# kyle-wedgwood/ArmadilloCUDALinearInterpolation

Hardware: NVIDIA B200
Metric: interp points/s (2-D bilinear, 4096x4096 f64 grid, 1e8 scattered queries) (higher is better)
Workload: dtype f64

## Files before the change

armadillocudalinearinterpolation_b200/csrc/host_staging.cuh:

```cuda
#pragma once
#include <cstdlib>
#include <cstring>
#include <string>
#include <thread>
#include <vector>
#include "common.cuh"

namespace b200 {

inline bool host_pageable(const void* p) {
  if (!p) return false;
  cudaPointerAttributes a;
  if (cudaPointerGetAttributes(&a, p) != cudaSuccess) { cudaGetLastError(); return true; }
  return a.type == cudaMemoryTypeUnregistered;
}

struct StageArray { const void* in; void* out; size_t elem; };

struct StagePool {
  static constexpr int kSlots = 2;
  struct Worker {
    cudaStream_t st = nullptr;
    cudaEvent_t ev[kSlots] = {nullptr, nullptr};
    std::vector<void*> pin[kSlots], dev[kSlots];
  };
  std::vector<Worker> workers;
  std::vector<size_t> elems;
  size_t chunk = 0;
  int device = -1;

  void release() {
    if (device >= 0) cudaSetDevice(device);
    for (Worker& w : workers) {
      for (int s = 0; s < kSlots; ++s) {
        for (void* p : w.pin[s]) cudaFreeHost(p);
        for (void* p : w.dev[s]) cudaFree(p);
        if (w.ev[s]) cudaEventDestroy(w.ev[s]);
      }
      if (w.st) cudaStreamDestroy(w.st);
    }
    workers.clear(); elems.clear(); chunk = 0;
  }
  ~StagePool() { release(); }

  int ensure(int dev_id, int nworkers, size_t chunk_elems, const std::vector<StageArray>& arrays) {
    bool same = device == dev_id && (int)workers.size() == nworkers && chunk == chunk_elems && elems.size() == arrays.size();
    for (size_t a = 0; same && a < arrays.size(); ++a) same = elems[a] == arrays[a].elem;
    if (same) return B200_OK;
    release();
    const int rc = build(dev_id, nworkers, chunk_elems, arrays);
    if (rc != B200_OK) release();
    return rc;
  }

  int build(int dev_id, int nworkers, size_t chunk_elems, const std::vector<StageArray>& arrays) {
    device = dev_id;
    chunk = chunk_elems;
    for (const StageArray& a : arrays) elems.push_back(a.elem);
    workers.resize(nworkers);
    for (Worker& w : workers) {
      B200_CUDA(cudaStreamCreateWithFlags(&w.st, cudaStreamNonBlocking));
      for (int s = 0; s < kSlots; ++s) {
        B200_CUDA(cudaEventCreateWithFlags(&w.ev[s], cudaEventDisableTiming));
        for (size_t e : elems) {
          void *hp = nullptr, *dp = nullptr;
          B200_CUDA(cudaHostAlloc(&hp, chunk * e, cudaHostAllocDefault));
          w.pin[s].push_back(hp);
          B200_CUDA(cudaMalloc(&dp, chunk * e));
          w.dev[s].push_back(dp);
        }
      }
    }
    return B200_OK;
  }
};

template <class Launch>
int staged_run(StagePool& pool, int device, const std::vector<StageArray>& arrays, size_t n, Launch launch) {
  if (n == 0) return B200_OK;
  constexpr size_t kChunkElems = (size_t)1 << 20;
  unsigned hw = std::thread::hardware_concurrency();
  int nworkers = (int)(hw >= 16 ? 8 : (hw >= 4 ? hw / 2 : 1));
  const size_t nchunks = (n + kChunkElems - 1) / kChunkElems;
  if ((size_t)nworkers > nchunks) nworkers = (int)nchunks;
  B200_TRY(pool.ensure(device, nworkers, kChunkElems, arrays));
  std::vector<int> status(nworkers, B200_OK);
  std::vector<std::string> text(nworkers);
  auto body = [&](int t) {
    auto run = [&]() -> int {
      B200_CUDA(cudaSetDevice(device));
      StagePool::Worker& w = pool.workers[t];
      bool pending[StagePool::kSlots] = {false, false};
      size_t p_off[StagePool::kSlots] = {0, 0}, p_cnt[StagePool::kSlots] = {0, 0};
      auto drain = [&](int s) -> int {
        if (!pending[s]) return B200_OK;
        B200_CUDA(cudaEventSynchronize(w.ev[s]));
        for (size_t a = 0; a < arrays.size(); ++a)
          if (arrays[a].out) memcpy((char*)arrays[a].out + p_off[s] * arrays[a].elem, w.pin[s][a], p_cnt[s] * arrays[a].elem);
        pending[s] = false;
        return B200_OK;
      };
      int slot = 0;
      for (size_t c = (size_t)t; c < nchunks; c += (size_t)nworkers, slot ^= 1) {
        const size_t off = c * kChunkElems, cnt = n - off < kChunkElems ? n - off : kChunkElems;
        B200_TRY(drain(slot));
        NvtxRange nvtx_chunk("staged:chunk memcpy+h2d+kernel+d2h");
        for (size_t a = 0; a < arrays.size(); ++a)
          if (arrays[a].in) {
            memcpy(w.pin[slot][a], (const char*)arrays[a].in + off * arrays[a].elem, cnt * arrays[a].elem);
            B200_CUDA(cudaMemcpyAsync(w.dev[slot][a], w.pin[slot][a], cnt * arrays[a].elem, cudaMemcpyHostToDevice, w.st));
          }
        B200_TRY(launch(w.dev[slot], cnt, w.st));
        for (size_t a = 0; a < arrays.size(); ++a)
          if (arrays[a].out)
            B200_CUDA(cudaMemcpyAsync(w.pin[slot][a], w.dev[slot][a], cnt * arrays[a].elem, cudaMemcpyDeviceToHost, w.st));
        B200_CUDA(cudaEventRecord(w.ev[slot], w.st));
        pending[slot] = true; p_off[slot] = off; p_cnt[slot] = cnt;
      }
      for (int s = 0; s < StagePool::kSlots; ++s) B200_TRY(drain(s));
      return B200_OK;
    };
    status[t] = run();
    if (status[t] != B200_OK) text[t] = b200_last_error();
  };
  std::vector<std::thread> th;
  bool spawn_failed = false;
  try {
    for (int t = 1; t < nworkers; ++t) th.emplace_back(body, t);
  } catch (...) {
    spawn_failed = true;
  }
  body(0);
  for (std::thread& x : th) x.join();
  if (spawn_failed) return fail(B200_ERR_CUDA, "staged copy: could not start the worker threads");
  for (int t = 0; t < nworkers; ++t)
    if (status[t] != B200_OK) return fail(status[t], "%s", text[t].c_str());
  return B200_OK;
}

}
```

Before: 55.91 billion.

## Replace per-call staging threads with persistent piece-scheduled pool and streaming copies

Replaces the per-call spawning of worker threads, each owning two slots, with a persistent thread pool. The pool shares six slots, each with its own stream, and splits chunks into pieces scheduled by a state machine (in, gpu, out), using cudaLaunchHostFunc callbacks to mark GPU completion. Host copies into and out of pinned buffers use AVX2/SSE2 non-temporal stores, and the thread count follows CPU affinity up to 16. This aims to remove thread creation cost and to overlap the host memcpy, the PCIe transfers and the kernels more fully. In exchange it adds mutex and condition-variable contention, a std::function call per launch, and considerable scheduling complexity.

Result: no change. 55.90 billion, median of 6 (-0.0%).

```diff
diff --git a/armadillocudalinearinterpolation_b200/csrc/host_staging.cuh b/armadillocudalinearinterpolation_b200/csrc/host_staging.cuh
--- a/armadillocudalinearinterpolation_b200/csrc/host_staging.cuh
+++ b/armadillocudalinearinterpolation_b200/csrc/host_staging.cuh
@@ -1,9 +1,16 @@
 #pragma once
+#include <sched.h>
+#include <condition_variable>
 #include <cstdlib>
 #include <cstring>
+#include <functional>
+#include <mutex>
 #include <string>
 #include <thread>
 #include <vector>
+#if defined(__x86_64__)
+#include <immintrin.h>
+#endif
 #include "common.cuh"
 
 namespace b200 {
@@ -15,61 +22,311 @@
   return a.type == cudaMemoryTypeUnregistered;
 }
 
+#if defined(__x86_64__)
+__attribute__((target("avx2"))) inline void stream_body_avx2(char* d, const char* s, size_t n) {
+  for (; n; n -= 128, d += 128, s += 128) {
+    const __m256i a = _mm256_loadu_si256((const __m256i*)s), b = _mm256_loadu_si256((const __m256i*)(s + 32)),
+                  c = _mm256_loadu_si256((const __m256i*)(s + 64)), e = _mm256_loadu_si256((const __m256i*)(s + 96));
+    _mm256_stream_si256((__m256i*)d, a);
+    _mm256_stream_si256((__m256i*)(d + 32), b);
+    _mm256_stream_si256((__m256i*)(d + 64), c);
+    _mm256_stream_si256((__m256i*)(d + 96), e);
+  }
+}
+inline void stream_body_sse2(char* d, const char* s, size_t n) {
+  for (; n; n -= 64, d += 64, s += 64) {
+    const __m128i a = _mm_loadu_si128((const __m128i*)s), b = _mm_loadu_si128((const __m128i*)(s + 16)),
+                  c = _mm_loadu_si128((const __m128i*)(s + 32)), e = _mm_loadu_si128((const __m128i*)(s + 48));
+    _mm_stream_si128((__m128i*)d, a);
+    _mm_stream_si128((__m128i*)(d + 16), b);
+    _mm_stream_si128((__m128i*)(d + 32), c);
+    _mm_stream_si128((__m128i*)(d + 48), e);
+  }
+}
+#endif
+
+inline void stream_copy(void* dst, const void* src, size_t n) {
+#if defined(__x86_64__)
+  static const bool avx2 = (__builtin_cpu_init(), __builtin_cpu_supports("avx2"));
+  char* d = (char*)dst;
+  const char* s = (const char*)src;
+  const size_t head = (32 - ((uintptr_t)d & 31)) & 31;
+  if (n < head + 128) { memcpy(d, s, n); return; }
+  memcpy(d, s, head);
+  d += head; s += head; n -= head;
+  const size_t body = n & ~(size_t)127;
+  if (avx2) stream_body_avx2(d, s, body);
+  else stream_body_sse2(d, s, body);
+  memcpy(d + body, s + body, n - body);
+#else
+  memcpy(dst, src, n);
+#endif
+}
+inline void stream_fence() {
+#if defined(__x86_64__)
+  _mm_sfence();
+#endif
+}
+
+inline int affinity_cpus() {
+  cpu_set_t set;
+  if (sched_getaffinity(0, sizeof(set), &set) == 0) return CPU_COUNT(&set);
+  const unsigned hw = std::thread::hardware_concurrency();
+  return hw ? (int)hw : 1;
+}
+
 struct StageArray { const void* in; void* out; size_t elem; };
 
+using StageLaunch = std::function<int(const std::vector<void*>&, size_t, cudaStream_t)>;
+
 struct StagePool {
-  static constexpr int kSlots = 2;
-  struct Worker {
-    cudaStream_t st = nullptr;
-    cudaEvent_t ev[kSlots] = {nullptr, nullptr};
-    std::vector<void*> pin[kSlots], dev[kSlots];
+  int max_threads = 16;
+  int nslots = 6;
+  size_t chunk_elems = (size_t)2 << 20;
+  size_t piece_elems = (size_t)1 << 19;
+
+  struct Slot { cudaStream_t st = nullptr; void* pin = nullptr; void* dev = nullptr; };
+  std::vector<Slot> slots;
+  size_t slot_bytes = 0;
+  int device = -1;
+
+  enum { kFree, kIn, kGpu, kOut };
+  struct Run { size_t chunk = 0, off = 0, cnt = 0; int state = kFree, pieces = 0, in_given = 0, in_done = 0,
+               out_given = 0, out_done = 0; };
+  struct Job;
+  struct Done { StagePool* pool; Job* job; int slot; };
+  struct Job {
+    const std::vector<StageArray>* arrays;
+    size_t n, nchunks;
+    int device;
+    const StageLaunch* launch;
+    std::vector<size_t> offs;
+    std::vector<Run> run;
+    std::vector<Done> done;
+    size_t next_chunk = 0, chunks_done = 0;
+    int status = B200_OK;
+    std::string text;
   };
-  std::vector<Worker> workers;
-  std::vector<size_t> elems;
-  size_t chunk = 0;
-  int device = -1;
-
+  enum { kTaskNone, kTaskIn, kTaskOut };
+  struct Task { int kind = kTaskNone, slot = 0, piece = 0; };
+
+  std::vector<std::thread> threads;
+  std::mutex mu;
+  std::condition_variable cv;
+  Job* job = nullptr;
+  unsigned long long job_id = 0;
+  int busy = 0;
+  bool quit = false;
+
+  StagePool() = default;
+  StagePool(const StagePool&) = delete;
+  StagePool& operator=(const StagePool&) = delete;
+  ~StagePool() { release(); }
+
+  void join_threads() {
+    {
+      std::lock_guard<std::mutex> lk(mu);
+      quit = true;
+    }
+    cv.notify_all();
+    for (std::thread& t : threads) t.join();
+    threads.clear();
+    quit = false;
+  }
+  void free_slots() {
+    if (device >= 0) cudaSetDevice(device);
+    for (Slot& s : slots) {
+      if (s.st) cudaStreamSynchronize(s.st);
+      if (s.pin) cudaFreeHost(s.pin);
+      if (s.dev) cudaFree(s.dev);
+      if (s.st) cudaStreamDestroy(s.st);
+    }
+    slots.clear();
+    slot_bytes = 0;
+  }
   void release() {
-    if (device >= 0) cudaSetDevice(device);
-    for (Worker& w : workers) {
-      for (int s = 0; s < kSlots; ++s) {
-        for (void* p : w.pin[s]) cudaFreeHost(p);
-        for (void* p : w.dev[s]) cudaFree(p);
-        if (w.ev[s]) cudaEventDestroy(w.ev[s]);
-      }
-      if (w.st) cudaStreamDestroy(w.st);
-    }
-    workers.clear(); elems.clear(); chunk = 0;
-  }
-  ~StagePool() { release(); }
-
-  int ensure(int dev_id, int nworkers, size_t chunk_elems, const std::vector<StageArray>& arrays) {
-    bool same = device == dev_id && (int)workers.size() == nworkers && chunk == chunk_elems && elems.size() == arrays.size();
-    for (size_t a = 0; same && a < arrays.size(); ++a) same = elems[a] == arrays[a].elem;
-    if (same) return B200_OK;
-    release();
-    const int rc = build(dev_id, nworkers, chunk_elems, arrays);
-    if (rc != B200_OK) release();
+    join_threads();
+    free_slots();
+  }
+
+  int ensure_slots(int dev_id, size_t bytes) {
+    if (device == dev_id && (int)slots.size() == nslots && slot_bytes >= bytes) return B200_OK;
+    free_slots();
+    device = dev_id;
+    const int rc = build_slots(bytes);
+    if (rc != B200_OK) free_slots();
     return rc;
   }
-
-  int build(int dev_id, int nworkers, size_t chunk_elems, const std::vector<StageArray>& arrays) {
-    device = dev_id;
-    chunk = chunk_elems;
-    for (const StageArray& a : arrays) elems.push_back(a.elem);
-    workers.resize(nworkers);
-    for (Worker& w : workers) {
-      B200_CUDA(cudaStreamCreateWithFlags(&w.st, cudaStreamNonBlocking));
-      for (int s = 0; s < kSlots; ++s) {
-        B200_CUDA(cudaEventCreateWithFlags(&w.ev[s], cudaEventDisableTiming));
-        for (size_t e : elems) {
-          void *hp = nullptr, *dp = nullptr;
-          B200_CUDA(cudaHostAlloc(&hp, chunk * e, cudaHostAllocDefault));
-          w.pin[s].push_back(hp);
-          B200_CUDA(cudaMalloc(&dp, chunk * e));
-          w.dev[s].push_back(dp);
-        }
-      }
+  int build_slots(size_t bytes) {
+    slots.resize(nslots);
+    for (Slot& s : slots) {
+      B200_CUDA(cudaStreamCreateWithFlags(&s.st, cudaStreamNonBlocking));
+      B200_CUDA(cudaHostAlloc(&s.pin, bytes, cudaHostAllocDefault));
+      B200_CUDA(cudaMalloc(&s.dev, bytes));
+    }
+    slot_bytes = bytes;
+    return B200_OK;
+  }
+
+  int ensure_threads(int want) {
+    try {
+      while ((int)threads.size() < want - 1) threads.emplace_back([this] { thread_main(); });
+    } catch (...) {
+      return fail(B200_ERR_CUDA, "staged copy: could not start the worker threads");
+    }
+    return B200_OK;
+  }
+
+  void thread_main() {
+    std::unique_lock<std::mutex> lk(mu);
+    unsigned long long seen = 0;
+    for (;;) {
+      cv.wait(lk, [&] { return quit || (job && job_id != seen); });
+      if (quit) return;
+      seen = job_id;
+      Job* j = job;
+      ++busy;
+      work(*j, lk);
+      --busy;
+      cv.notify_all();
+    }
+  }
+
+  Task pick(Job& j) {
+    Task t;
+    const int S = (int)j.run.size();
+    auto oldest = [&](auto pred) {
+      int best = -1;
+      for (int s = 0; s < S; ++s)
+        if (pred(j.run[s]) && (best < 0 || j.run[s].chunk < j.run[best].chunk)) best = s;
+      return best;
+    };
+    int s = oldest([](const Run& r) { return r.state == kOut && r.out_given < r.pieces; });
+    if (s >= 0) { t.kind = kTaskOut; t.slot = s; t.piece = j.run[s].out_given++; return t; }
+    while (j.next_chunk < j.nchunks && j.run[j.next_chunk % S].state == kFree) {
+      Run& r = j.run[j.next_chunk % S];
+      r = Run();
+      r.chunk = j.next_chunk++;
+      r.off = r.chunk * chunk_elems;
+      r.cnt = j.n - r.off < chunk_elems ? j.n - r.off : chunk_elems;
+      r.pieces = (int)((r.cnt + piece_elems - 1) / piece_elems);
+      r.state = kIn;
+    }
+    s = oldest([](const Run& r) { return r.state == kIn && r.in_given < r.pieces; });
+    if (s >= 0) { t.kind = kTaskIn; t.slot = s; t.piece = j.run[s].in_given++; }
+    return t;
+  }
+
+  void work(Job& j, std::unique_lock<std::mutex>& lk) {
+    lk.unlock();
+    const cudaError_t e = cudaSetDevice(j.device);
+    lk.lock();
+    if (e != cudaSuccess) {
+      cuda_fail(e, "cudaSetDevice", __FILE__, __LINE__);
+      if (j.status == B200_OK) { j.status = B200_ERR_CUDA; j.text = b200_last_error(); }
+      cv.notify_all();
+      return;
+    }
+    for (;;) {
+      if (j.status != B200_OK || j.chunks_done == j.nchunks) return;
+      const Task t = pick(j);
+      if (t.kind == kTaskNone) { cv.wait(lk); continue; }
+      Run& r = j.run[t.slot];
+      lk.unlock();
+      bool launch = false;
+      int rc = run_task(j, t, r, lk, launch);
+      if (rc == B200_OK && launch) rc = enqueue_gpu(j, t.slot, r);
+      const std::string text = rc != B200_OK ? b200_last_error() : "";
+      lk.lock();
+      if (rc != B200_OK && j.status == B200_OK) { j.status = rc; j.text = text; }
+      cv.notify_all();
+    }
+  }
+
+  int run_task(Job& j, const Task& t, Run& r, std::unique_lock<std::mutex>& lk, bool& launch) {
+    const std::vector<StageArray>& arrays = *j.arrays;
+    Slot& sl = slots[t.slot];
+    const size_t p0 = (size_t)t.piece * piece_elems;
+    const size_t cnt = r.cnt - p0 < piece_elems ? r.cnt - p0 : piece_elems;
+    const size_t off = r.off + p0;
+    if (t.kind == kTaskIn) {
+      for (size_t a = 0; a < arrays.size(); ++a)
+        if (arrays[a].in) stream_copy((char*)sl.pin + j.offs[a] + p0 * arrays[a].elem,
+                                      (const char*)arrays[a].in + off * arrays[a].elem, cnt * arrays[a].elem);
+      stream_fence();
+      for (size_t a = 0; a < arrays.size(); ++a)
+        if (arrays[a].in)
+          B200_CUDA(cudaMemcpyAsync((char*)sl.dev + j.offs[a] + p0 * arrays[a].elem,
+                                    (char*)sl.pin + j.offs[a] + p0 * arrays[a].elem, cnt * arrays[a].elem,
+                                    cudaMemcpyHostToDevice, sl.st));
+      std::lock_guard<std::mutex> g(*lk.mutex());
+      launch = ++r.in_done == r.pieces;
+      if (launch) r.state = kGpu;
+      return B200_OK;
+    }
+    for (size_t a = 0; a < arrays.size(); ++a)
+      if (arrays[a].out) stream_copy((char*)arrays[a].out + off * arrays[a].elem,
+                                     (const char*)sl.pin + j.offs[a] + p0 * arrays[a].elem, cnt * arrays[a].elem);
+    stream_fence();
+    std::lock_guard<std::mutex> g(*lk.mutex());
+    if (++r.out_done == r.pieces) { r.state = kFree; ++j.chunks_done; }
+    return B200_OK;
+  }
+
+  int enqueue_gpu(Job& j, int s, const Run& r) {
+    const std::vector<StageArray>& arrays = *j.arrays;
+    Slot& sl = slots[s];
+    std::vector<void*> d(arrays.size());
+    for (size_t a = 0; a < arrays.size(); ++a) d[a] = (char*)sl.dev + j.offs[a];
+    B200_TRY((*j.launch)(d, r.cnt, sl.st));
+    for (size_t a = 0; a < arrays.size(); ++a)
+      if (arrays[a].out)
+        B200_CUDA(cudaMemcpyAsync((char*)sl.pin + j.offs[a], d[a], r.cnt * arrays[a].elem, cudaMemcpyDeviceToHost,
+                                  sl.st));
+    B200_CUDA(cudaLaunchHostFunc(sl.st, gpu_done, &j.done[s]));
+    return B200_OK;
+  }
+
+  static void CUDART_CB gpu_done(void* arg) {
+    const Done* d = (const Done*)arg;
+    std::lock_guard<std::mutex> g(d->pool->mu);
+    d->job->run[d->slot].state = kOut;
+    d->pool->cv.notify_all();
+  }
+
+  int run(int dev_id, const std::vector<StageArray>& arrays, size_t n, const StageLaunch& launch) {
+    if (n == 0) return B200_OK;
+    Job j;
+    j.arrays = &arrays;
+    j.n = n;
+    j.nchunks = (n + chunk_elems - 1) / chunk_elems;
+    j.device = dev_id;
+    j.launch = &launch;
+    size_t bytes = 0;
+    for (const StageArray& a : arrays) {
+      j.offs.push_back(bytes);
+      bytes += (chunk_elems * a.elem + 4095) & ~(size_t)4095;
+    }
+    B200_TRY(ensure_slots(dev_id, bytes));
+    j.run.resize(slots.size());
+    for (int s = 0; s < (int)slots.size(); ++s) j.done.push_back({this, &j, s});
+    const size_t items = j.nchunks * ((chunk_elems + piece_elems - 1) / piece_elems);
+    int want = affinity_cpus();
+    if (want > max_threads) want = max_threads;
+    if ((size_t)want > items) want = (int)items;
+    B200_TRY(ensure_threads(want));
+    std::unique_lock<std::mutex> lk(mu);
+    job = &j;
+    ++job_id;
+    cv.notify_all();
+    work(j, lk);
+    cv.wait(lk, [&] { return busy == 0; });
+    job = nullptr;
+    lk.unlock();
+    if (j.status != B200_OK) {
+      for (Slot& s : slots) cudaStreamSynchronize(s.st);
+      cudaGetLastError();
+      return fail(j.status, "%s", j.text.c_str());
     }
     return B200_OK;
   }
@@ -77,65 +334,7 @@
 
 template <class Launch>
 int staged_run(StagePool& pool, int device, const std::vector<StageArray>& arrays, size_t n, Launch launch) {
-  if (n == 0) return B200_OK;
-  constexpr size_t kChunkElems = (size_t)1 << 20;
-  unsigned hw = std::thread::hardware_concurrency();
-  int nworkers = (int)(hw >= 16 ? 8 : (hw >= 4 ? hw / 2 : 1));
-  const size_t nchunks = (n + kChunkElems - 1) / kChunkElems;
-  if ((size_t)nworkers > nchunks) nworkers = (int)nchunks;
-  B200_TRY(pool.ensure(device, nworkers, kChunkElems, arrays));
-  std::vector<int> status(nworkers, B200_OK);
-  std::vector<std::string> text(nworkers);
-  auto body = [&](int t) {
-    auto run = [&]() -> int {
-      B200_CUDA(cudaSetDevice(device));
-      StagePool::Worker& w = pool.workers[t];
-      bool pending[StagePool::kSlots] = {false, false};
-      size_t p_off[StagePool::kSlots] = {0, 0}, p_cnt[StagePool::kSlots] = {0, 0};
-      auto drain = [&](int s) -> int {
-        if (!pending[s]) return B200_OK;
-        B200_CUDA(cudaEventSynchronize(w.ev[s]));
-        for (size_t a = 0; a < arrays.size(); ++a)
-          if (arrays[a].out) memcpy((char*)arrays[a].out + p_off[s] * arrays[a].elem, w.pin[s][a], p_cnt[s] * arrays[a].elem);
-        pending[s] = false;
-        return B200_OK;
-      };
-      int slot = 0;
-      for (size_t c = (size_t)t; c < nchunks; c += (size_t)nworkers, slot ^= 1) {
-        const size_t off = c * kChunkElems, cnt = n - off < kChunkElems ? n - off : kChunkElems;
-        B200_TRY(drain(slot));
-        NvtxRange nvtx_chunk("staged:chunk memcpy+h2d+kernel+d2h");
-        for (size_t a = 0; a < arrays.size(); ++a)
-          if (arrays[a].in) {
-            memcpy(w.pin[slot][a], (const char*)arrays[a].in + off * arrays[a].elem, cnt * arrays[a].elem);
-            B200_CUDA(cudaMemcpyAsync(w.dev[slot][a], w.pin[slot][a], cnt * arrays[a].elem, cudaMemcpyHostToDevice, w.st));
-          }
-        B200_TRY(launch(w.dev[slot], cnt, w.st));
-        for (size_t a = 0; a < arrays.size(); ++a)
-          if (arrays[a].out)
-            B200_CUDA(cudaMemcpyAsync(w.pin[slot][a], w.dev[slot][a], cnt * arrays[a].elem, cudaMemcpyDeviceToHost, w.st));
-        B200_CUDA(cudaEventRecord(w.ev[slot], w.st));
-        pending[slot] = true; p_off[slot] = off; p_cnt[slot] = cnt;
-      }
-      for (int s = 0; s < StagePool::kSlots; ++s) B200_TRY(drain(s));
-      return B200_OK;
-    };
-    status[t] = run();
-    if (status[t] != B200_OK) text[t] = b200_last_error();
-  };
-  std::vector<std::thread> th;
-  bool spawn_failed = false;
-  try {
-    for (int t = 1; t < nworkers; ++t) th.emplace_back(body, t);
-  } catch (...) {
-    spawn_failed = true;
-  }
-  body(0);
-  for (std::thread& x : th) x.join();
-  if (spawn_failed) return fail(B200_ERR_CUDA, "staged copy: could not start the worker threads");
-  for (int t = 0; t < nworkers; ++t)
-    if (status[t] != B200_OK) return fail(status[t], "%s", text[t].c_str());
-  return B200_OK;
-}
-
-}
+  return pool.run(device, arrays, n, StageLaunch(launch));
+}
+
+}
```
